# baiyang4/D-LSG-Video-Caption

Measured on AMD Instinct MI355X. Metric: clips/sec (train step, 26x(2048+4096) feats), higher is better.
Workload: dtype f32; 1 GPU; vocab 1000, dropout on, tf eps 0.952, batch 64/GPU; MSVD-shaped 26x(2048+4096) + 16x2048 regions; train step; batch_per_gpu=64, global_batch=64, parallelism=dp1, launch=hipGraph replay, gemm_arithmetic=fp32

## Files before the change

d-lsg-video-caption_amd/csrc/gemm.hip:

```cpp
#include <cstdlib>
#include <mutex>

#include "common.hpp"
#include "dlsg.h"

namespace {

constexpr int NT = 256;

template <int ROWS, bool T, int BK>
struct TileGeom {
    static constexpr int NV = ROWS * BK / 4 / NT;
    static constexpr int LD = T ? (ROWS + 4) : (BK + 4);
    static constexpr int ELEMS = T ? BK * (ROWS + 4) : ROWS * (BK + 4);
    static constexpr int KQ = BK / 4;
};

template <int ROWS, bool T, int BK>
__device__ __forceinline__ void load_tile_fast(const float* __restrict__ base, int64_t ld, int row0, int k0, int rmax,
                                               f32x4 (&regs)[TileGeom<ROWS, T, BK>::NV]) {
    constexpr int NV = TileGeom<ROWS, T, BK>::NV;
#pragma unroll
    for (int j = 0; j < NV; ++j) {
        const int f = threadIdx.x + NT * j;
// ... 538 lines not shown
    const bool accum = p.flags & DLSG_GEMM_ACCUM, use_bias = (p.flags & DLSG_GEMM_BIAS) && biasp != nullptr;
    const bool do_tanh = p.flags & DLSG_GEMM_TANH;
#pragma unroll
    for (int nj = 0; nj < NJ; ++nj) {
        const int col = n0 + 32 * nj + r;
        if (col >= N) continue;
        const float bv = use_bias ? biasp[col] : 0.f;
#pragma unroll
        for (int mi = 0; mi < MI; ++mi)
#pragma unroll
            for (int ee = 0; ee < 4; ++ee) {
                const int e = 4 * w + ee;
                const int row = 32 * mi + (e & 3) + 8 * (e >> 2) + 4 * h;
                if (row >= M) continue;
                float v = 0.f;
#pragma unroll
                for (int ww = 0; ww < 4; ++ww) v += red[(((ww * MI + mi) * NJ + nj) * 16 + e) * 64 + lane];
                v = p.alpha * v + bv;
                float* cp = C + (int64_t)row * (grp.ldc ? grp.ldc : (int64_t)p.ldc) + col;
                if (accum) v += *cp;
                if (do_tanh) v = tanhf(v);
                *cp = v;
            }
    }
}

template <int MI>
int launch_skinny_mi(const dlsg_gemm_args* a, const KArgs& k, hipStream_t st) {
    dim3 grid((a->N + 31) / 32, a->ngroups * a->nbatch, 1), block(NT, 1, 1);
    static std::once_flag once;
    std::call_once(once, [] {
        (void)hipFuncSetAttribute(reinterpret_cast<const void*>(&skinny2_nt_kernel<MI, 1>), hipFuncAttributeMaxDynamicSharedMemorySize,
                                  s2_lds_bytes(MI, 1));
        (void)hipFuncSetAttribute(reinterpret_cast<const void*>(&skinny2_nt_kernel<MI, 2>), hipFuncAttributeMaxDynamicSharedMemorySize,
                                  s2_lds_bytes(MI, 2));
        (void)hipFuncSetAttribute(reinterpret_cast<const void*>(&skinny2_nt_kernel<MI, 1, true>), hipFuncAttributeMaxDynamicSharedMemorySize,
                                  s2_lds_bytes(MI, 1));
        (void)hipFuncSetAttribute(reinterpret_cast<const void*>(&skinny2_nt_kernel<MI, 2, true>), hipFuncAttributeMaxDynamicSharedMemorySize,
                                  s2_lds_bytes(MI, 2));
        (void)hipFuncSetAttribute(reinterpret_cast<const void*>(&skinny_kernel<false, MI>), hipFuncAttributeMaxDynamicSharedMemorySize,
                                  skinny_lds_bytes(MI));
        (void)hipFuncSetAttribute(reinterpret_cast<const void*>(&skinny_kernel<true, MI>), hipFuncAttributeMaxDynamicSharedMemorySize,
                                  skinny_lds_bytes(MI));
    });
    if (a->mode == 0) {
        bool ok = a->nbatch == 1;
        for (int i = 0; i < a->ngroups && ok; ++i) {
            const dlsg_gemm_group& g = a->g[i];
            ok = (g.K % 4 == 0) && g.K >= S2_STAGE && (g.lda % 4 == 0) && (g.ldb % 4 == 0) &&
                 ((reinterpret_cast<uintptr_t>(g.A) & 15) == 0) && ((reinterpret_cast<uintptr_t>(g.B) & 15) == 0);
        }
        if (ok) {
            const int wg64 = ((a->N + 63) / 64) * a->ngroups * a->nbatch;
            if (wg64 >= 224) {
                dim3 grid2((a->N + 63) / 64, a->ngroups * a->nbatch, 1);
                hipLaunchKernelGGL((skinny2_nt_kernel<MI, 2>), grid2, block, s2_lds_bytes(MI, 2), st, k);
            } else {
                hipLaunchKernelGGL((skinny2_nt_kernel<MI, 1>), grid, block, s2_lds_bytes(MI, 1), st, k);
            }
        } else {
            hipLaunchKernelGGL((skinny_kernel<false, MI>), grid, block, skinny_lds_bytes(MI), st, k);
        }
    } else {
        bool ok = a->nbatch == 1;
        for (int i = 0; i < a->ngroups && ok; ++i) {
            const dlsg_gemm_group& g = a->g[i];
            const int gn = g.N > 0 ? g.N : a->N;
            ok = (g.K % 4 == 0) && g.K >= S2_STAGE && (g.lda % 4 == 0) && (g.ldb % 4 == 0) && (gn % 4 == 0) && gn >= 4 &&
                 ((reinterpret_cast<uintptr_t>(g.A) & 15) == 0) && ((reinterpret_cast<uintptr_t>(g.B) & 15) == 0);
        }
        if (ok) {
            bool same_n = true;
            for (int i = 0; i < a->ngroups; ++i) same_n = same_n && (a->g[i].N == 0 || a->g[i].N == a->N);
            const int wg64 = ((a->N + 63) / 64) * a->ngroups * a->nbatch;
            if (wg64 >= 224 && same_n) {
                dim3 grid2((a->N + 63) / 64, a->ngroups * a->nbatch, 1);
                hipLaunchKernelGGL((skinny2_nt_kernel<MI, 2, true>), grid2, block, s2_lds_bytes(MI, 2), st, k);
            } else {
                hipLaunchKernelGGL((skinny2_nt_kernel<MI, 1, true>), grid, block, s2_lds_bytes(MI, 1), st, k);
            }
        } else {
            hipLaunchKernelGGL((skinny_kernel<true, MI>), grid, block, skinny_lds_bytes(MI), st, k);
        }
    }
    DLSG_CHECK_LAUNCH();
    return DLSG_OK;
}

int launch_skinny(const dlsg_gemm_args* a, hipStream_t st) {
    KArgs k;
    k.M = a->M; k.N = a->N; k.ldc = a->ldc; k.ngroups = a->ngroups; k.flags = a->flags;
    k.bsa = a->bsa; k.bsb = a->bsb; k.bsc = a->bsc; k.alpha = a->alpha; k.bias = a->bias; k.skip_if = a->skip_if;
    for (int i = 0; i < a->ngroups; ++i) k.g[i] = a->g[i];
    return a->M <= 64 ? launch_skinny_mi<2>(a, k, st) : launch_skinny_mi<4>(a, k, st);
}

template <int BM, int BN, int BK>
int launch(const dlsg_gemm_args* a, hipStream_t st) {
    KArgs k;
    k.M = a->M; k.N = a->N; k.ldc = a->ldc; k.ngroups = a->ngroups; k.flags = a->flags;
    k.bsa = a->bsa; k.bsb = a->bsb; k.bsc = a->bsc; k.alpha = a->alpha; k.bias = a->bias; k.skip_if = a->skip_if;
    for (int i = 0; i < a->ngroups; ++i) k.g[i] = a->g[i];
    const int tiles = ((a->M + BM - 1) / BM) * ((a->N + BN - 1) / BN);
    dim3 grid(tiles, a->ngroups * a->nbatch, 1), block(NT, 1, 1);
    switch (a->mode) {
        case 0:
            if constexpr (BM == 128) hipLaunchKernelGGL((gemm_kernel_w3<BM, BN, false, false, BK>), grid, block, 0, st, k);
            else hipLaunchKernelGGL((gemm_kernel<BM, BN, false, false, BK>), grid, block, 0, st, k);
            break;
        case 1:
            if constexpr (BM == 128) hipLaunchKernelGGL((gemm_kernel_w3<BM, BN, false, true, BK>), grid, block, 0, st, k);
            else hipLaunchKernelGGL((gemm_kernel<BM, BN, false, true, BK>), grid, block, 0, st, k);
            break;
        case 2:
            if constexpr (BM == 128) hipLaunchKernelGGL((gemm_kernel_w3<BM, BN, true, true, BK>), grid, block, 0, st, k);
            else hipLaunchKernelGGL((gemm_kernel<BM, BN, true, true, BK>), grid, block, 0, st, k);
            break;
        default: return DLSG_EINVAL;
    }
    DLSG_CHECK_LAUNCH();
    return DLSG_OK;
}

__global__ void slab_reduce_kernel(const float* __restrict__ slabs, int nslab, int64_t stride,
                                   const float* __restrict__ bias, float* __restrict__ out, int64_t rows, int n,
                                   int ldo, int flags) {
    const int64_t total = rows * n;
    for (int64_t i = (int64_t)blockIdx.x * blockDim.x + threadIdx.x; i < total; i += (int64_t)gridDim.x * blockDim.x) {
        const int64_t rrow = i / n;
        const int col = (int)(i - rrow * n);
        float s = 0.f;
        int k = 0;
        for (; k + 4 <= nslab; k += 4) {
            const float t0 = slabs[k * stride + i], t1 = slabs[(k + 1) * stride + i], t2 = slabs[(k + 2) * stride + i],
                        t3 = slabs[(k + 3) * stride + i];
            s += t0; s += t1; s += t2; s += t3;
        }
        for (; k < nslab; ++k) s += slabs[k * stride + i];
        if ((flags & DLSG_GEMM_BIAS) && bias) s += bias[col];
        float* op = out + rrow * ldo + col;
        if (flags & DLSG_GEMM_ACCUM) s += *op;
        if (flags & DLSG_GEMM_TANH) s = tanhf(s);
        *op = s;
    }
}

}

int dlsg_gemm_bf16x3_dispatch(const dlsg_gemm_args* a, hipStream_t st);
int dlsg_gemm_big_ok(const dlsg_gemm_args* a);
int dlsg_gemm_big_dispatch(const dlsg_gemm_args* a, hipStream_t st, int bn);
int dlsg_gemm_sk_wanted(const dlsg_gemm_args* a);
int dlsg_gemm_sk_dispatch(const dlsg_gemm_args* a, hipStream_t st);

extern "C" int dlsg_abi_version(void) { return DLSG_ABI_VERSION; }

static int gemm_plan(const dlsg_gemm_args* a, int64_t* m1_out) {
    const int64_t z = (int64_t)a->ngroups * a->nbatch;
    const int64_t tilesL = (int64_t)((a->M + 127) / 128) * ((a->N + 127) / 128) * z;
    if (a->flags & DLSG_GEMM_SK) return DLSG_GEMM_V_SK;
    if (a->flags & DLSG_GEMM_TILE256) return (a->flags & DLSG_GEMM_FORCE128) ? DLSG_GEMM_V_256x128 : DLSG_GEMM_V_256;
    if ((a->flags & (DLSG_GEMM_FORCE64 | DLSG_GEMM_FORCE128)) == (DLSG_GEMM_FORCE64 | DLSG_GEMM_FORCE128))
        return DLSG_GEMM_V_128x64;
    if (a->flags & DLSG_GEMM_FORCE64) return DLSG_GEMM_V_64;
    if (a->flags & DLSG_GEMM_FORCE128) return DLSG_GEMM_V_128;
    if (a->M <= 128 && a->mode != 2 && a->N >= 64) return DLSG_GEMM_V_SKINNY;
    if (dlsg_gemm_sk_wanted(a)) return DLSG_GEMM_V_SK;
    if (tilesL >= 1000) {
        bool plain = dlsg_gemm_big_ok(a) != 0;
        for (int i = 0; i < a->ngroups && plain; ++i) plain = a->g[i].N == 0 || a->g[i].N == a->N;
        const int64_t pad_n = (a->N + 255) / 256 * 256;
        if (plain && pad_n * 10 <= (int64_t)a->N * 11) {
            const int64_t panel = (pad_n / 256) * z;
            int64_t g = panel, b = 256;
            while (b) { const int64_t t = g % b; g = b; b = t; }
            const int64_t need = 256 / g;
            const int64_t m1 = (a->M / 256) / need * need * 256;
            if (m1 == a->M) return DLSG_GEMM_V_256;
            if (m1 > 0 && (a->M - m1) * 4 <= a->M) {
                if (m1_out) *m1_out = m1;
                return DLSG_GEMM_V_256_HEAD;
            }
        }
        return DLSG_GEMM_V_128;
    }
    const int padM = (a->M + 127) / 128 * 128;
    if ((padM - a->M) * 10 <= a->M) {
        if (tilesL >= 500 && a->mode == 2) return DLSG_GEMM_V_128;
        if (tilesL >= 200) return DLSG_GEMM_V_128x64;
    }
    return DLSG_GEMM_V_64;
}

static bool gemm_args_ok(const dlsg_gemm_args* a) {
    return a && a->ngroups >= 1 && a->ngroups <= DLSG_GEMM_MAXG && a->nbatch >= 1 && a->M >= 0 && a->N >= 0 &&
           (int64_t)a->ngroups * a->nbatch <= 65535;
}

extern "C" int dlsg_gemm_variant(const dlsg_gemm_args* a) {
    if (!gemm_args_ok(a)) return DLSG_EINVAL;
    if (a->flags & DLSG_GEMM_BF16X3) return DLSG_EINVAL;
    return gemm_plan(a, nullptr);
}

extern "C" int dlsg_gemm(const dlsg_gemm_args* a, void* stream) {
    if (!gemm_args_ok(a)) return DLSG_EINVAL;
    if (a->M == 0 || a->N == 0) return DLSG_OK;
    hipStream_t st = reinterpret_cast<hipStream_t>(stream);
    if (a->flags & DLSG_GEMM_BF16X3) return dlsg_gemm_bf16x3_dispatch(a, st);
    int64_t m1 = 0;
    switch (gemm_plan(a, &m1)) {
        case DLSG_GEMM_V_SK: return dlsg_gemm_sk_dispatch(a, st);
        case DLSG_GEMM_V_256: return dlsg_gemm_big_dispatch(a, st, 256);
        case DLSG_GEMM_V_256x128: return dlsg_gemm_big_dispatch(a, st, 128);
        case DLSG_GEMM_V_256_HEAD: {
            dlsg_gemm_args head = *a, tail = *a;
            head.M = (int)m1;
            tail.M = a->M - (int)m1;
            for (int i = 0; i < a->ngroups; ++i) {
                const int64_t ldc = a->g[i].ldc ? a->g[i].ldc : (int64_t)a->ldc;
                tail.g[i].A = a->g[i].A + (a->mode == 2 ? m1 : m1 * a->g[i].lda);
                tail.g[i].C = a->g[i].C + m1 * ldc;
            }
            const int rc = dlsg_gemm_big_dispatch(&head, st, 256);
            return rc != DLSG_OK ? rc : dlsg_gemm(&tail, stream);
        }
        case DLSG_GEMM_V_SKINNY: return launch_skinny(a, st);
        case DLSG_GEMM_V_128: return launch<128, 128, 32>(a, st);
        case DLSG_GEMM_V_128x64: return launch<128, 64, 64>(a, st);
        default: return launch<64, 64, 64>(a, st);
    }
}

extern "C" int dlsg_slab_reduce(const float* slabs, int nslab, int64_t slab_stride, const float* bias, float* out,
                                int64_t rows, int n, int ldo, int flags, void* stream) {
    if (!slabs || !out || nslab < 1) return DLSG_EINVAL;
    const int64_t total = rows * n;
    if (total == 0) return DLSG_OK;
    int blocks = (int)((total + 255) / 256);
    if (blocks > 2048) blocks = 2048;
    hipLaunchKernelGGL(slab_reduce_kernel, dim3(blocks), dim3(256), 0, reinterpret_cast<hipStream_t>(stream), slabs,
                       nslab, slab_stride, bias, out, rows, n, ldo, flags);
    DLSG_CHECK_LAUNCH();
    return DLSG_OK;
}
```

d-lsg-video-caption_amd/dlsg_amd/hip.py:

```python
import ctypes as C
import math
import os

import torch

from . import abi

_HERE = os.path.dirname(os.path.abspath(__file__))
LIB_PATH = os.path.join(_HERE, 'libdlsg_hip.so')

_D = abi.defines
ABI_VERSION = _D['DLSG_ABI_VERSION']
MAXG = _D['DLSG_GEMM_MAXG']
SAMPLE_FILTER_MAXV = _D['DLSG_SAMPLE_FILTER_MAXV']
GEMM_NT, GEMM_NN, GEMM_TN = _D['DLSG_GEMM_NT'], _D['DLSG_GEMM_NN'], _D['DLSG_GEMM_TN']
F_ACCUM, F_BIAS, F_TANH = _D['DLSG_GEMM_ACCUM'], _D['DLSG_GEMM_BIAS'], _D['DLSG_GEMM_TANH']
F_FORCE64, F_FORCE128, F_TILE256, F_BF16X3 = (_D['DLSG_GEMM_' + n] for n in ('FORCE64', 'FORCE128', 'TILE256', 'BF16X3'))
F_SK, F_NOSK, F_SK_BM128, F_SK_BM256, F_SK_BN128, F_SK_NOXMAP = (_D['DLSG_GEMM_' + n] for n in (
    'SK', 'NOSK', 'SK_BM128', 'SK_BM256', 'SK_BN128', 'SK_NOXMAP'))
GRAD_SUMSQ_SLOTS = _D['DLSG_GRAD_SUMSQ_SLOTS']
CLIP_NORM, CLIP_COEF, CLIP_NONFINITE, CLIP_RECORD_FLOATS = (_D['DLSG_CLIP_' + n] for n in ('NORM', 'COEF', 'NONFINITE', 'RECORD_FLOATS'))
ENS_MAX = _D['DLSG_ENS_MAX']
METRICS_STAGE = _D['DLSG_METRICS_STAGE']
F_SK_GIVEAWAY = _D['DLSG_GEMM_SK_GIVEAWAY']

i64, u32, u64, f32 = C.c_int64, C.c_uint32, C.c_uint64, C.c_float


def load_library(path=LIB_PATH):
    if not os.path.exists(path):
        raise RuntimeError('libdlsg_hip.so not built (%s): run `python -c "import __graft_entry__ as g; g.build()"` '
                           'or `make -C d-lsg-video-caption_amd/csrc`; there is no fallback path' % path)
    lib = C.CDLL(path)
    for name, (restype, argtypes) in abi.functions.items():
        fn = getattr(lib, name)
        fn.restype, fn.argtypes = restype, argtypes
    if lib.dlsg_abi_version() != ABI_VERSION:
        raise RuntimeError('libdlsg_hip.so ABI mismatch: library %d, include/dlsg.h %d (rebuild: make -C d-lsg-video-caption_amd/csrc)'
                           % (lib.dlsg_abi_version(), ABI_VERSION))
    return lib




def _p(t):
    return None if t is None else C.c_void_p(t.data_ptr())


def _chkc(t):
    if not t.is_contiguous():
        raise ValueError('fused decoder-step kernels take dense row-major buffers')


def _seed(seed):
    if torch.is_tensor(seed):
        return 0, C.c_void_p(seed.data_ptr())
    return int(seed), None


def cider_tables(tb):
    def p(t):
        return t.data_ptr() if t.numel() else None
    return abi.dlsg_cider_tables(p(tb.gram_keys), p(tb.gram_idf), p(tb.clip_off), p(tb.ref_off), p(tb.ref_norm), p(tb.ref_len),
                                 p(tb.ent_keys), p(tb.ent_w), tb.gram_keys.numel(), tb.log_n, tb.sigma, tb.n_clips, tb.V, tb.n, 0)


def host_to_device(values, dtype, device):
    t = values.to(dtype) if torch.is_tensor(values) else torch.as_tensor(values, dtype=dtype)
    device = torch.device(device)
    if device.type != 'cuda' or t.is_cuda:
        return t.to(device)
    return t.contiguous().pin_memory().to(device, non_blocking=True)


def copy_to_device(dst, values, dtype=None):
    t = values.to(dtype or dst.dtype) if torch.is_tensor(values) else torch.as_tensor(values, dtype=dtype or dst.dtype)
    if dst.is_cuda and not t.is_cuda:
        t = t.contiguous().pin_memory()
    dst.copy_(t.view(dst.shape), non_blocking=True)


def normalised_weights(weights):
    w = [float(x) for x in weights]
    if not w or not all(math.isfinite(x) and x > 0.0 for x in w):
        raise ValueError('ensemble weights must be finite and positive, not %r' % (list(weights),))
    tot = math.fsum(w)
    return [x / tot for x in w]


def _chk2(t):
    assert t.dim() == 2 and (t.stride(1) == 1 or t.size(1) == 1) and t.dtype == torch.float32, (t.shape, t.stride())
    return t


class HipOps(object):

    name = 'hip'

    def __init__(self):
        self.lib = load_library()
        if not torch.cuda.is_available():
            raise RuntimeError('dlsg_amd needs an MI355X (gfx950) device: torch.cuda.is_available() is False and '
                               'there is no CPU fallback')
        self.prof = None
        self.extra_flags = 0
        self.prof_min_flops = 2e9
        self.flop_count = None
        self._tail_ws = {}

    def _prof_begin(self):
        if self.prof is None:
            return None
        e0 = torch.cuda.Event(enable_timing=True)
        e0.record()
        return e0

    def _prof_end(self, key, e0, work, shape='', operand_bytes=None):
        if e0 is None:
            return
        e1 = torch.cuda.Event(enable_timing=True)
        e1.record()
        self.prof.setdefault(key, []).append((e0, e1, work, shape, operand_bytes))

    def prof_summary(self):
        out = {}
        for key, rec in (self.prof or {}).items():
            shapes, samples = {}, {}
            for a, b, w, shp, ob in rec:
                d = shapes.setdefault(shp, dict(launches=0, ms_total=0.0, work_total=0.0, operand_bytes=ob))
                d['launches'] += 1; d['work_total'] += float(w)
                samples.setdefault(shp, []).append(a.elapsed_time(b))
            for shp, ms in samples.items():
                ms = sorted(ms)
                med = ms[len(ms) // 2] if len(ms) % 2 else 0.5 * (ms[len(ms) // 2 - 1] + ms[len(ms) // 2])
                shapes[shp]['ms_total'] = med * len(ms)
            out[key] = dict(launches=len(rec), ms_total=sum(d['ms_total'] for d in shapes.values()),
                            work_total=float(sum(r[2] for r in rec)), shapes=shapes)
        return out

    @staticmethod
    def _stream():
        return C.c_void_p(torch.cuda.current_stream().cuda_stream)

    launches = 0

    def _check(self, rc, what):
        self.launches += 1
        if rc != 0:
            raise RuntimeError('%s failed with code %d' % (what, rc))

    stream_k = True
    sk_cu_budget = 0

    _gemm_ws = {}
    _capture_streams = {}

    @classmethod
    def capture_stream(cls, dev):
        dev = torch.device(dev)
        idx = dev.index if dev.index is not None else torch.cuda.current_device()
        st = cls._capture_streams.get(idx)
        if st is None:
            st = cls._capture_streams[idx] = torch.cuda.Stream(device=idx)
        return st

    def _gemm_workspace(self, dev):
        key = (dev.index, torch.cuda.current_stream(dev).cuda_stream)
        ws = HipOps._gemm_ws.get(key)
        if ws is None:
            n = int(self.lib.dlsg_gemm_ws_bytes())
            if n <= 0:
                raise RuntimeError('dlsg_gemm_ws_bytes() failed: no device?')
            if torch.cuda.is_current_stream_capturing():
                return None
            ws = HipOps._gemm_ws[key] = torch.zeros((n + 3) // 4, dtype=torch.float32, device=dev)
        return ws
# ... 1235 lines not shown
```

include/dlsg.h:

```cpp
#ifndef DLSG_H
#define DLSG_H
#include <stdint.h>
#ifdef __cplusplus
extern "C" {
#endif

#define DLSG_ABI_VERSION 8
int dlsg_abi_version(void);

#define DLSG_OK 0
#define DLSG_EINVAL (-1)
#define DLSG_ELAUNCH (-2)
#define DLSG_EALIGN (-3)
#define DLSG_ENOCOMM (-4)
int dlsg_struct_size(int which);

#define DLSG_GEMM_NT 0
#define DLSG_GEMM_NN 1
#define DLSG_GEMM_TN 2
#define DLSG_GEMM_MAXG 16
#define DLSG_GEMM_ACCUM 1
#define DLSG_GEMM_BIAS 2
#define DLSG_GEMM_TANH 4
#define DLSG_GEMM_FORCE64 256
#define DLSG_GEMM_FORCE128 512
#define DLSG_GEMM_TILE256 2048
#define DLSG_GEMM_SK 4096
#define DLSG_GEMM_NOSK 8192
#define DLSG_GEMM_SK_BM128 16384
#define DLSG_GEMM_SK_BM256 32768
#define DLSG_GEMM_SK_BN128 262144
#define DLSG_GEMM_SK_NOXMAP 131072
#define DLSG_GEMM_SK_GIVEAWAY 65536
#define DLSG_GEMM_BF16X3 1024
typedef struct {
    const float* A;
    const float* B;
    float* C;
    int64_t lda, ldb;
    int32_t K;
    int32_t N;
    const float* bias;
    int64_t ldc;
} dlsg_gemm_group;
typedef struct {
    int32_t mode, M, N, ldc;
    int32_t ngroups, nbatch, flags;
    int32_t cu_budget;
    int64_t bsa, bsb, bsc;
    float alpha;
    int32_t pad2_;
    const float* bias;
    const int32_t* skip_if;
    void* ws;
    int64_t ws_bytes;
    int32_t* err;
    dlsg_gemm_group g[DLSG_GEMM_MAXG];
} dlsg_gemm_args;
int dlsg_gemm(const dlsg_gemm_args* args, void* stream);
int64_t dlsg_gemm_ws_bytes(void);
#define DLSG_GEMM_V_64 0
#define DLSG_GEMM_V_128x64 1
#define DLSG_GEMM_V_128 2
#define DLSG_GEMM_V_SKINNY 3
#define DLSG_GEMM_V_256 4
#define DLSG_GEMM_V_256x128 5
#define DLSG_GEMM_V_256_HEAD 6
#define DLSG_GEMM_V_SK 7
int dlsg_gemm_variant(const dlsg_gemm_args* args);

int dlsg_slab_reduce(const float* slabs, int nslab, int64_t slab_stride, const float* bias, float* out,
                     int64_t rows, int n, int ldo, int flags, void* stream);

typedef struct {
    const float* x; int64_t ldx;
    const float* res; int64_t ldres;
    const float* gamma; const float* beta;
    float* y; int64_t ldy;
    float* stats;
    const float* pe; int32_t pe_rows;
    int32_t rows, n;
    int32_t pre_tanh, post_tanh;
    float eps;
    float p1, p2;
    uint64_t seed; uint32_t site1, site2;
    const uint64_t* seed_ptr;
} dlsg_rowln_args;
int dlsg_rowln_fwd(const dlsg_rowln_args* a, void* stream);
#define DLSG_ROWLN_MAXMULTI 2
int dlsg_rowln_fwd_multi(const dlsg_rowln_args* a, int count, void* stream);
typedef struct {
    dlsg_rowln_args f;
    const float* dy; int64_t lddy;
    float* dx; int64_t lddx;
    int32_t accum_dx;
    float* dgb_part; int32_t nblk;
} dlsg_rowln_bwd_args;
int dlsg_rowln_bwd(const dlsg_rowln_bwd_args* a, void* stream);
int dlsg_rowln_bwd_multi(const dlsg_rowln_bwd_args* a, int count, void* stream);
int dlsg_rowln_bwd_nblk(int rows);
int64_t dlsg_colsum_ws_floats(int rows, int n);
int dlsg_colsum(const float* part, int64_t ld, int rows, int n, float* out, int accum, float* ws, void* stream);
int dlsg_colsum2(const float* part, int64_t ld, int rows, int n, float* out_a, float* out_b, int split, int dup, int accum,
                 float* ws, void* stream);
#define DLSG_COLSUM_MAXMULTI 32
typedef struct {
    const float* part; int64_t ld;
    float* out_a; float* out_b;
    int32_t rows, n, split, dup, accum, pad_;
} dlsg_colsum_desc;
int dlsg_colsum_multi_ok(const float* part, int64_t ld, int rows, int n);
int dlsg_colsum_multi(const dlsg_colsum_desc* d, int count, void* stream);

typedef struct {
    const float* y; const float* v;
    const float* g_obj; const float* b_obj;
    float* z;
    float* ml;
    float* ostats;
    float* S;
    float* ws; int64_t ws_bytes;
    int32_t B, T, NO, H, nsplit;
    float scale, eps;
} dlsg_o2v_args;
int64_t dlsg_o2v_workspace_bytes(int B, int T, int H, int nsplit);
int dlsg_o2v_fwd(const dlsg_o2v_args* a, void* stream);
#define DLSG_O2V_MAXMULTI 2
int dlsg_o2v_fwd_multi(const dlsg_o2v_args* a, int count, void* stream);
typedef struct {
    const float* y; const float* ostats; const float* g_obj; const float* b_obj;
    const float* v; const float* z; const float* dz; const float* S; const float* ml;
    float* pd; float* m12;
    float* dy; float* dv; float* part;
    float* ws; int64_t ws_bytes;
    int32_t B, T, NO, H, nsplit;
    float scale;
    float* dysum;
} dlsg_o2v_bwd_args;
int dlsg_o2v_bwd_multi(const dlsg_o2v_bwd_args* a, int count, void* stream);
int dlsg_o2v_bwd(const dlsg_o2v_bwd_args* a, void* stream);

typedef struct {
    const float* ov; const float* theta; const float* gamma; const float* beta;
    float* adj; float* u; float* out; float* stats;
    int32_t B, T, P, H;
    float p; uint32_t site; float eps; float pad_;
    uint64_t seed; const uint64_t* seed_ptr;
} dlsg_latent_psl_args;
int dlsg_latent_psl_fwd(const dlsg_latent_psl_args* a, void* stream);
#define DLSG_PSL_MAXMULTI 2
int dlsg_latent_psl_fwd_multi(const dlsg_latent_psl_args* a, int count, void* stream);
typedef struct {
    const float* dout; const float* u; const float* stats; const float* gamma;
    const float* adj; const float* ov; const float* theta;
    float* dov; float* dtheta_part; float* part;
    int32_t B, T, P, H;
    float p; uint32_t site;
    uint64_t seed; const uint64_t* seed_ptr;
} dlsg_latent_psl_bwd_args;
int dlsg_latent_psl_bwd(const dlsg_latent_psl_bwd_args* a, void* stream);
int dlsg_latent_psl_bwd_multi(const dlsg_latent_psl_bwd_args* a, int count, void* stream);

typedef struct {
    const float* K; const float* Q; const float* V; const float* mask;
    float* w; float* out;
    int32_t B, T, D; float scale;
} dlsg_sa_core_args;
int dlsg_sa_core_fwd(const dlsg_sa_core_args* a, void* stream);
typedef struct {
    const float* w; const float* K; const float* Q; const float* V; const float* dout;
    float* dK; float* dQ; float* dV;
    int32_t B, T, D; float scale;
} dlsg_sa_core_bwd_args;
int dlsg_sa_core_bwd(const dlsg_sa_core_bwd_args* a, void* stream);

int dlsg_softmax_fwd(const float* x, const float* mask, float* y, int64_t outer, int n, int inner, void* stream);
int dlsg_softmax_bwd(const float* y, const float* dy, float* dx, int64_t outer, int n, int inner, void* stream);

typedef struct {
    const float* Kp[2]; const float* Vp[2];
    const float* q; int64_t ldq;
    float* c[2]; int64_t ldc;
    float* alpha;
    int32_t B, P, Q, H, nstream;
    float scale;
} dlsg_decatt_args;
// ... 390 lines not shown
```

Measured before the change: 5071 clips/s.

## Add async direct-to-LDS pipelined fp32 MFMA GEMM for tiled variants

Adds a second-generation tiled GEMM kernel that loads A/B tiles straight into LDS with global_load_lds_dwordx4, uses a 2-3 stage ring of buffers and interleaves fragment reads and next-stage issues with fp32 MFMA 32x32x2 instructions. It also uses a swizzled LDS layout to avoid bank conflicts. The 64x64, 128x64 and 128x128 dispatch paths now route to it whenever alignment and shape checks pass, and a new flag keeps the old kernels reachable. The aim is to hide global memory latency and raise MFMA utilisation. In exchange it relies on inline asm and hand-set waitcnt counts, which could cause correctness or occupancy problems.

```diff
diff --git a/d-lsg-video-caption_amd/csrc/gemm.hip b/d-lsg-video-caption_amd/csrc/gemm.hip
--- a/d-lsg-video-caption_amd/csrc/gemm.hip
+++ b/d-lsg-video-caption_amd/csrc/gemm.hip
@@ -714,6 +714,8 @@
 int dlsg_gemm_big_dispatch(const dlsg_gemm_args* a, hipStream_t st, int bn);
 int dlsg_gemm_sk_wanted(const dlsg_gemm_args* a);
 int dlsg_gemm_sk_dispatch(const dlsg_gemm_args* a, hipStream_t st);
+int dlsg_gemm_tile2_ok(const dlsg_gemm_args* a, int variant);
+int dlsg_gemm_tile2_dispatch(const dlsg_gemm_args* a, hipStream_t st, int variant);
 
 extern "C" int dlsg_abi_version(void) { return DLSG_ABI_VERSION; }
 
@@ -765,6 +767,15 @@
     return gemm_plan(a, nullptr);
 }
 
+static int launch_tile(const dlsg_gemm_args* a, hipStream_t st, int variant) {
+    if (!(a->flags & DLSG_GEMM_TILE_GEN1) && dlsg_gemm_tile2_ok(a, variant)) return dlsg_gemm_tile2_dispatch(a, st, variant);
+    switch (variant) {
+        case DLSG_GEMM_V_128: return launch<128, 128, 32>(a, st);
+        case DLSG_GEMM_V_128x64: return launch<128, 64, 64>(a, st);
+        default: return launch<64, 64, 64>(a, st);
+    }
+}
+
 extern "C" int dlsg_gemm(const dlsg_gemm_args* a, void* stream) {
     if (!gemm_args_ok(a)) return DLSG_EINVAL;
     if (a->M == 0 || a->N == 0) return DLSG_OK;
@@ -788,9 +799,9 @@
             return rc != DLSG_OK ? rc : dlsg_gemm(&tail, stream);
         }
         case DLSG_GEMM_V_SKINNY: return launch_skinny(a, st);
-        case DLSG_GEMM_V_128: return launch<128, 128, 32>(a, st);
-        case DLSG_GEMM_V_128x64: return launch<128, 64, 64>(a, st);
-        default: return launch<64, 64, 64>(a, st);
+        case DLSG_GEMM_V_128: return launch_tile(a, st, DLSG_GEMM_V_128);
+        case DLSG_GEMM_V_128x64: return launch_tile(a, st, DLSG_GEMM_V_128x64);
+        default: return launch_tile(a, st, DLSG_GEMM_V_64);
     }
 }
 
diff --git a/d-lsg-video-caption_amd/csrc/gemm_tile2.hip b/d-lsg-video-caption_amd/csrc/gemm_tile2.hip
--- /dev/null
+++ b/d-lsg-video-caption_amd/csrc/gemm_tile2.hip
@@ -0,0 +1,290 @@
+#include <mutex>
+#include <type_traits>
+
+#include "common.hpp"
+#include "dlsg.h"
+
+namespace {
+
+constexpr int T2_THREADS = 256;
+constexpr int T2_BK = 32;
+
+struct T2Args {
+    int M, N, ldc, ngroups, flags;
+    int64_t bsa, bsb, bsc;
+    float alpha;
+    const float* bias;
+    const int32_t* skip_if;
+    dlsg_gemm_group g[DLSG_GEMM_MAXG];
+};
+
+typedef __attribute__((address_space(3))) void* t2_lp_t;
+
+__device__ __forceinline__ void t2_glds16(const char* base, uint32_t voff, uint32_t lds_addr) {
+#if defined(__HIP_DEVICE_COMPILE__)
+    asm volatile("s_mov_b32 m0, %0\n\tglobal_load_lds_dwordx4 %1, %2" : : "s"(lds_addr), "v"(voff), "s"(base) : "memory", "m0");
+#endif
+}
+__device__ __forceinline__ int t2_u(int x) { return __builtin_amdgcn_readfirstlane(x); }
+__device__ __forceinline__ const char* t2_up(const void* q) {
+    const uint64_t u = reinterpret_cast<uint64_t>(q);
+    const uint32_t lo = __builtin_amdgcn_readfirstlane((uint32_t)u), hi = __builtin_amdgcn_readfirstlane((uint32_t)(u >> 32));
+    return reinterpret_cast<const char*>(((uint64_t)hi << 32) | lo);
+}
+
+template <bool T, int ROWS>
+__device__ __forceinline__ void t2_voff(uint32_t (&voff)[ROWS / 32], uint32_t (&tail)[ROWS / 32], int w, int lane, int row0,
+                                        int rmax, int64_t ld, int rem) {
+    constexpr int PW = ROWS / 32;
+#pragma unroll
+    for (int i = 0; i < PW; ++i) {
+        const int pc = w * PW + i;
+        if (!T) {
+            const int R = 8 * pc + (lane >> 3);
+            const int seg = (lane & 7) ^ ((R >> 1) & 7);
+            const uint32_t row = (uint32_t)((min(row0 + R, rmax - 1) - row0) * ld * 4);
+            voff[i] = row + 16 * seg;
+            tail[i] = row + 16 * min(seg, max(rem / 4 - 1, 0));
+        } else {
+            constexpr int KR = 256 / ROWS, LPR = 64 / KR;
+            const int kr = KR * pc + lane / LPR;
+            const uint32_t col = (min(row0 + 4 * (lane % LPR), rmax - 4) - row0) * 4;
+            voff[i] = (uint32_t)(kr * ld * 4) + col;
+            tail[i] = (uint32_t)(min(kr, rem - 1) * ld * 4) + col;
+        }
+    }
+}
+
+template <int BM, int BN, bool AT, bool BT, int D>
+__global__ __launch_bounds__(T2_THREADS) void gemm_tile2_kernel(const T2Args p) {
+    constexpr int TM = BM / 64, TNB = BN / 64;
+    constexpr int WM = BM / 2, WN = BN / 2;
+    constexpr int ABYTES = BM * 128, BBYTES = BN * 128, STAGE = ABYTES + BBYTES;
+    constexpr int PA = BM / 32, PB = BN / 32, PT = PA + PB;
+    static_assert(PT <= 4 * TM, "a stage's pieces are issued one per MFMA slot of g3");
+    static_assert(TM + TNB <= 4 * TM, "one fragment read per MFMA slot");
+    extern __shared__ __attribute__((aligned(16))) char t2_lds[];
+
+    const int tiles_n = (p.N + BN - 1) / BN;
+    int tm, z, tn;
+    dlsg::gemm_tile_map(tiles_n, tm, z, tn);
+    const int m0 = tm * BM, n0 = tn * BN;
+
+    if (p.skip_if && *p.skip_if) return;
+    const int gi = z % p.ngroups, bi = z / p.ngroups;
+    const dlsg_gemm_group grp = p.g[gi];
+    const float* A = grp.A + (int64_t)bi * p.bsa;
+    const float* B = grp.B + (int64_t)bi * p.bsb;
+    float* C = grp.C + (int64_t)bi * p.bsc;
+    const int K = grp.K;
+    const int Ng = grp.N > 0 ? grp.N : p.N;
+    if (n0 >= Ng) return;
+
+    const int lane = threadIdx.x & 63;
+    const int w = t2_u(threadIdx.x >> 6);
+    const int r = lane & 31, h = lane >> 5;
+    const int wm = w >> 1, wn = w & 1;
+    const uint32_t lds0 = t2_u((uint32_t)reinterpret_cast<uintptr_t>((t2_lp_t)t2_lds));
+
+    f32x16 acc[TM][TNB];
+#pragma unroll
+    for (int i = 0; i < TM; ++i)
+#pragma unroll
+        for (int j = 0; j < TNB; ++j)
+#pragma unroll
+            for (int e = 0; e < 16; ++e) acc[i][j][e] = 0.f;
+
+    const int nst = (K + T2_BK - 1) / T2_BK;
+    const int rem = K - T2_BK * (nst - 1);
+    uint32_t voffA[PA], voffB[PB], tailA[PA], tailB[PB];
+    t2_voff<AT, BM>(voffA, tailA, w, lane, m0, p.M, grp.lda, rem);
+    t2_voff<BT, BN>(voffB, tailB, w, lane, n0, Ng, grp.ldb, rem);
+    const char* baseA = t2_up(AT ? A + m0 : A + (int64_t)m0 * grp.lda);
+    const char* baseB = t2_up(BT ? B + n0 : B + (int64_t)n0 * grp.ldb);
+    const int64_t strA = AT ? 4 * grp.lda : 4, strB = BT ? 4 * grp.ldb : 4;
+    auto issue = [&](int s, int buf, int pc) {
+        const int64_t kf = (int64_t)T2_BK * s;
+        const bool tl = s == nst - 1 && rem < T2_BK;
+        const uint32_t dst = lds0 + buf * STAGE;
+        if (pc < PA) t2_glds16(baseA + kf * strA, tl ? tailA[pc] : voffA[pc], dst + (w * PA + pc) * 1024);
+        else t2_glds16(baseB + kf * strB, tl ? tailB[pc - PA] : voffB[pc - PA], dst + ABYTES + (w * PB + (pc - PA)) * 1024);
+    };
+
+    int offA[4], offB[4];
+#pragma unroll
+    for (int g = 0; g < 4; ++g) {
+        const int ks = (4 * h + g) ^ ((r >> 1) & 7);
+        offA[g] = AT ? ((16 * h + 4 * g) * BM + wm * WM + r) * 4 : (wm * WM + r) * 128 + ks * 16;
+        offB[g] = ABYTES + (BT ? ((16 * h + 4 * g) * BN + wn * WN + r) * 4 : (wn * WN + r) * 128 + ks * 16);
+    }
+    f32x4 fa[2][TM], fb[2][TNB];
+    auto read_frag = [&](int buf, const char* st, int g, int f) {
+        if (f < TM) {
+            if (!AT) fa[buf][f] = *reinterpret_cast<const f32x4*>(st + offA[g] + f * 32 * 128);
+            else {
+#pragma unroll
+                for (int j = 0; j < 4; ++j) fa[buf][f][j] = *reinterpret_cast<const float*>(st + offA[g] + (j * BM + f * 32) * 4);
+            }
+        } else {
+            const int c = f - TM;
+            if (!BT) fb[buf][c] = *reinterpret_cast<const f32x4*>(st + offB[g] + c * 32 * 128);
+            else {
+#pragma unroll
+                for (int j = 0; j < 4; ++j) fb[buf][c][j] = *reinterpret_cast<const float*>(st + offB[g] + (j * BN + c * 32) * 4);
+            }
+        }
+    };
+
+#pragma unroll
+    for (int s = 0; s < D; ++s)
+        if (s < nst) {
+#pragma unroll
+            for (int pc = 0; pc < PT; ++pc) issue(s, s, pc);
+        }
+    if (nst >= D) asm volatile("s_waitcnt vmcnt(%0)" ::"n"((D - 1) * PT) : "memory");
+    else asm volatile("s_waitcnt vmcnt(0)" ::: "memory");
+    __builtin_amdgcn_s_barrier();
+    asm volatile("" ::: "memory");
+#pragma unroll
+    for (int f = 0; f < TM + TNB; ++f) read_frag(0, t2_lds, 0, f);
+
+    const int remh = rem - 16 * h;
+
+    int cbuf = 0;
+    auto stage = [&](auto mode_tag, int i) {
+        constexpr int MODE = decltype(mode_tag)::value;
+        const int nbuf = cbuf + 1 == D ? 0 : cbuf + 1;
+        const char* st = t2_lds + cbuf * STAGE;
+        const char* stn = t2_lds + nbuf * STAGE;
+#pragma unroll
+        for (int g = 0; g < 4; ++g) {
+            const int cur = g & 1, nxt = cur ^ 1;
+#pragma unroll
+            for (int s = 0; s < 4 * TM; ++s) {
+                const int j = s / TM, ti = s % TM;
+                float av = fa[cur][ti][j];
+                if (MODE == 2) av = (4 * g + j < remh) ? av : 0.f;
+#pragma unroll
+                for (int jn = 0; jn < TNB; ++jn) {
+                    float bv = fb[cur][jn][j];
+                    if (MODE == 2) bv = (4 * g + j < remh) ? bv : 0.f;
+                    acc[ti][jn] = __builtin_amdgcn_mfma_f32_32x32x2f32(av, bv, acc[ti][jn], 0, 0, 0);
+                }
+                if (s < TM + TNB) {
+                    if (g < 3) read_frag(nxt, st, g + 1, s);
+                    else if (MODE != 2) read_frag(nxt, stn, 0, s);
+                }
+                if (MODE == 0 && g == 3 && s < PT) issue(i + D, cbuf, s);
+                __builtin_amdgcn_sched_barrier(0);
+            }
+            if (g == 2 && MODE != 2) {
+                if (MODE == 0) asm volatile("s_waitcnt vmcnt(%0) lgkmcnt(0)" ::"n"((D - 2) * PT) : "memory");
+                else asm volatile("s_waitcnt vmcnt(0) lgkmcnt(0)" ::: "memory");
+                __builtin_amdgcn_s_barrier();
+                asm volatile("" ::: "memory");
+                __builtin_amdgcn_sched_barrier(0);
+            }
+        }
+        cbuf = nbuf;
+    };
+    int i = 0;
+    for (; i + D < nst; ++i) stage(std::integral_constant<int, 0>{}, i);
+    for (; i + 1 < nst; ++i) stage(std::integral_constant<int, 1>{}, i);
+    stage(std::integral_constant<int, 2>{}, i);
+    asm volatile("s_waitcnt vmcnt(0)" ::: "memory");
+
+    const float* biasp = grp.bias ? grp.bias : p.bias;
+    const bool accum = p.flags & DLSG_GEMM_ACCUM, use_bias = (p.flags & DLSG_GEMM_BIAS) && biasp != nullptr;
+    const bool do_tanh = p.flags & DLSG_GEMM_TANH;
+#pragma unroll
+    for (int ti = 0; ti < TM; ++ti)
+#pragma unroll
+        for (int j = 0; j < TNB; ++j) {
+            const int col = n0 + wn * WN + j * 32 + r;
+            if (col >= Ng) continue;
+            const float bv = use_bias ? biasp[col] : 0.f;
+            const int64_t ldc = grp.ldc ? grp.ldc : (int64_t)p.ldc;
+            const int rbase = m0 + wm * WM + ti * 32 + 4 * h;
+            float* cp = C + (int64_t)rbase * ldc + col;
+            float oldv[16];
+#pragma unroll
+            for (int e = 0; e < 16; ++e) {
+                const int ro = (e & 3) + 8 * (e >> 2);
+                oldv[e] = (accum && rbase + ro < p.M) ? cp[(int64_t)ro * ldc] : 0.f;
+            }
+#pragma unroll
+            for (int e = 0; e < 16; ++e) {
+                const int ro = (e & 3) + 8 * (e >> 2);
+                if (rbase + ro >= p.M) continue;
+                float v = p.alpha * acc[ti][j][e] + bv + oldv[e];
+                if (do_tanh) v = tanhf(v);
+                cp[(int64_t)ro * ldc] = v;
+            }
+        }
+}
+
+constexpr int t2_depth(int bm, int bn) { return bm * bn >= 128 * 128 ? 2 : 3; }
+
+template <int BM, int BN, bool AT, bool BT, int D>
+int t2_launch(const T2Args& k, dim3 grid, hipStream_t st) {
+    constexpr int lds_bytes = D * (BM + BN) * 128;
+    static std::once_flag once;
+    static hipError_t attr_rc = hipSuccess;
+    std::call_once(once, [] {
+        attr_rc = hipFuncSetAttribute(reinterpret_cast<const void*>(&gemm_tile2_kernel<BM, BN, AT, BT, D>),
+                                      hipFuncAttributeMaxDynamicSharedMemorySize, lds_bytes);
+    });
+    if (attr_rc != hipSuccess) return DLSG_ELAUNCH;
+    hipLaunchKernelGGL((gemm_tile2_kernel<BM, BN, AT, BT, D>), grid, dim3(T2_THREADS), lds_bytes, st, k);
+    DLSG_CHECK_LAUNCH();
+    return DLSG_OK;
+}
+
+template <int BM, int BN>
+int t2_launch_mode(const dlsg_gemm_args* a, const T2Args& k, hipStream_t st) {
+    const int tiles = ((a->M + BM - 1) / BM) * ((a->N + BN - 1) / BN);
+    const dim3 grid(tiles, a->ngroups * a->nbatch, 1);
+    switch (a->mode) {
+        case 0: return t2_launch<BM, BN, false, false, t2_depth(BM, BN)>(k, grid, st);
+        case 1: return t2_launch<BM, BN, false, true, t2_depth(BM, BN)>(k, grid, st);
+        case 2: return t2_launch<BM, BN, true, true, t2_depth(BM, BN)>(k, grid, st);
+        default: return DLSG_EINVAL;
+    }
+}
+
+}
+
+int dlsg_gemm_tile2_ok(const dlsg_gemm_args* a, int variant) {
+    const bool at = a->mode == 2, bt = a->mode != 0;
+    if (a->mode < 0 || a->mode > 2) return 0;
+    if (variant == DLSG_GEMM_V_128) {
+        int kmax = 0;
+        for (int i = 0; i < a->ngroups; ++i) kmax = a->g[i].K > kmax ? a->g[i].K : kmax;
+        if (kmax <= 2 * T2_BK) return 0;
+    }
+    if (a->nbatch > 1 && ((a->bsa % 4) || (a->bsb % 4))) return 0;
+    if (at && (a->M < 4 || (a->M % 4))) return 0;
+    for (int i = 0; i < a->ngroups; ++i) {
+        const dlsg_gemm_group& g = a->g[i];
+        const int gn = g.N > 0 ? g.N : a->N;
+        if (g.K < T2_BK || (g.lda % 4) || (g.ldb % 4) || g.lda <= 0 || g.ldb <= 0) return 0;
+        if ((reinterpret_cast<uintptr_t>(g.A) & 15) || (reinterpret_cast<uintptr_t>(g.B) & 15)) return 0;
+        if (bt && (gn < 4 || (gn % 4))) return 0;
+        if ((g.K % T2_BK) && (g.K % 4) && !(at && bt)) return 0;
+        if ((int64_t)128 * g.lda * 4 >= (1LL << 31) || (int64_t)128 * g.ldb * 4 >= (1LL << 31)) return 0;
+    }
+    return 1;
+}
+
+int dlsg_gemm_tile2_dispatch(const dlsg_gemm_args* a, hipStream_t st, int variant) {
+    T2Args k;
+    k.M = a->M; k.N = a->N; k.ldc = a->ldc; k.ngroups = a->ngroups; k.flags = a->flags;
+    k.bsa = a->bsa; k.bsb = a->bsb; k.bsc = a->bsc; k.alpha = a->alpha; k.bias = a->bias; k.skip_if = a->skip_if;
+    for (int i = 0; i < a->ngroups; ++i) k.g[i] = a->g[i];
+    switch (variant) {
+        case DLSG_GEMM_V_128: return t2_launch_mode<128, 128>(a, k, st);
+        case DLSG_GEMM_V_128x64: return t2_launch_mode<128, 64>(a, k, st);
+        case DLSG_GEMM_V_64: return t2_launch_mode<64, 64>(a, k, st);
+        default: return DLSG_EINVAL;
+    }
+}
diff --git a/d-lsg-video-caption_amd/dlsg_amd/hip.py b/d-lsg-video-caption_amd/dlsg_amd/hip.py
--- a/d-lsg-video-caption_amd/dlsg_amd/hip.py
+++ b/d-lsg-video-caption_amd/dlsg_amd/hip.py
@@ -22,6 +22,7 @@
 CLIP_NORM, CLIP_COEF, CLIP_NONFINITE, CLIP_RECORD_FLOATS = (_D['DLSG_CLIP_' + n] for n in ('NORM', 'COEF', 'NONFINITE', 'RECORD_FLOATS'))
 ENS_MAX = _D['DLSG_ENS_MAX']
 METRICS_STAGE = _D['DLSG_METRICS_STAGE']
+F_TILE_GEN1 = _D['DLSG_GEMM_TILE_GEN1']
 F_SK_GIVEAWAY = _D['DLSG_GEMM_SK_GIVEAWAY']
 
 i64, u32, u64, f32 = C.c_int64, C.c_uint32, C.c_uint64, C.c_float
diff --git a/include/dlsg.h b/include/dlsg.h
--- a/include/dlsg.h
+++ b/include/dlsg.h
@@ -32,6 +32,7 @@
 #define DLSG_GEMM_SK_BN128 262144
 #define DLSG_GEMM_SK_NOXMAP 131072
 #define DLSG_GEMM_SK_GIVEAWAY 65536
+#define DLSG_GEMM_TILE_GEN1 524288
 #define DLSG_GEMM_BF16X3 1024
 typedef struct {
     const float* A;
```

Result: no change. 5104 clips/s, median of 6 (+0.6%).
